# fab-jul/L3C-PyTorch

Hardware: NVIDIA B200
Metric: Mpixels/s encode+decode (lossless round-trip) (higher is better)
Workload: dtype f16

## Files before the change

### include/l3c_b200.h

```cpp
#ifndef L3C_B200_H_
#define L3C_B200_H_

#include <stddef.h>
#include <stdint.h>

#ifdef __cplusplus
extern "C" {
#endif

#define L3C_OK 0
#define L3C_EINVAL (-1)
#define L3C_ECUDA (-2)
#define L3C_EOVERFLOW (-3)
#define L3C_ENODEV (-4)
#define L3C_EUNSUPPORTED (-5)

const char *l3c_last_error(void);
int l3c_version(void);

long long l3c_launch_log(char *buf, size_t cap, int reset);


int l3c_cuda_supported(void);

int l3c_encode_cdf(const uint16_t *cdf_host, int64_t n_sym, int Lp, const int16_t *sym_host,
                   uint8_t *out_host, size_t out_cap, size_t *out_len);

int l3c_decode_cdf(const uint16_t *cdf_host, int64_t n_sym, int Lp, const uint8_t *in_host,
                   size_t in_len, int16_t *sym_out_host);

int l3c_encode_logistic_mixture(const float *targets_dev, const float *means_dev,
                                const float *log_scales_dev, const float *probs_dev, int K,
                                int64_t n_sym, int Lp, const int16_t *sym_host,
                                uint8_t *out_host, size_t out_cap, size_t *out_len);

int l3c_decode_logistic_mixture(const float *targets_dev, const float *means_dev,
                                const float *log_scales_dev, const float *probs_dev, int K,
                                int64_t n_sym, int Lp, const uint8_t *in_host, size_t in_len,
                                int16_t *sym_out_host);


typedef struct {
    const uint32_t *intervals;
    uint8_t *out;
    uint32_t n_sym;
    uint32_t out_cap;
} l3c_enc_stream_t;

int l3c_ac_encode_streams(const l3c_enc_stream_t *streams_dev, int n_streams,
                          uint32_t *out_len_dev, void *stream);

typedef struct {
    const uint16_t *table;
    const uint8_t *in;
    uint8_t *sym_out;
    uint32_t *state;
    int64_t row_pitch;
    uint32_t n_sym;
    uint32_t in_len;
} l3c_dec_stream_t;

int l3c_ac_decode_streams(const l3c_dec_stream_t *streams_dev, int n_streams, int L,
                          uint32_t first, uint32_t count, void *stream);

int l3c_pack_streams(const l3c_enc_stream_t *streams_dev, const uint32_t *len_dev,
                     const uint64_t *dst_off_dev, int n_streams, uint8_t *blob_dev, void *stream);

int l3c_lut_intervals(const uint8_t *sym_dev, const uint32_t *lut_dev, int64_t n,
                      uint32_t *intervals_dev, void *stream);


int l3c_uniform_cdf_row(int L, uint16_t *row_host);

int l3c_dmll_intervals(const float *l_dev, const uint8_t *sym_dev, const float *targets_dev,
                       int N, int HW, int C, int K, int L, int rgb, uint32_t *intervals_dev,
                       void *stream);

int l3c_dmll_build_table(const float *l_dev, const uint8_t *sym_dev, const float *targets_dev,
                         int N, int HW, int C, int K, int L, int rgb, int c, int pix0, int npix,
                         uint16_t *table_dev, int pitch, void *stream);

int l3c_dmll_build_table_tiled(const float *l_dev, const uint8_t *sym_dev, const float *targets_dev,
                               int N, int H, int W, int C, int K, int L, int rgb, int c, int th, int tw,
                               uint16_t *table_dev, int pitch, void *stream);
int l3c_reorder_tiles(const void *src_dev, void *dst_dev, int elem_bytes, int planes, int H, int W, int th,
                      int tw, int to_tiles, void *stream);

int l3c_dmll_nll(const float *l_dev, const uint8_t *sym_dev, const float *values_dev,
                 int N, int HW, int C, int K, int L, int rgb, float x_min, float x_max,
                 double *nll_dev, float *nll_map_dev ,
                 void *stream);

int l3c_dmll_channel_params(const float *l_dev, const float *x_dec_dev, int N, int HW, int C, int K,
                            int rgb, int c, float *pi_dev, float *mu_dev, float *log_scales_dev,
                            void *stream);

int l3c_dmll_sample(const float *l_dev, const float *u_sel_dev, const float *u_x_dev, int N, int HW, int C, int K,
                    int rgb, float *x_dev, void *stream);


#define L3C_CONV_RELU 1u
#define L3C_CONV_PIXEL_SHUFFLE2 2u
#define L3C_CONV_ROUND_TF32 4u

#define L3C_PREC_FP32 0
#define L3C_PREC_TF32 1
#define L3C_PREC_F16 2
#define L3C_PREC_F16X2 3

typedef struct {
    const float *x;
    const float *w;
    const float *bias;
    const float *residual;
    float *y;
    float *y_tf32;
    void *y_h;
    const void *x_h;
    const void *w_h;
    int N, H, W, Cin, x_pitch;
    int Cout, cout_pad, y_pitch, y_coff;
    int ksize, stride, dilation;
    unsigned flags;
    int precision;
    int yh_pitch;
    int yh_lo_off;
} l3c_conv_t;

int l3c_conv2d(const l3c_conv_t *p, void *stream);

int l3c_lin_dmll_intervals(const void *x_h, const void *w_h, const float *bias, const uint8_t *sym_dev,
                           const float *targets_dev, int N, int HW, int Cin, int C, int K, int L, int rgb,
                           uint32_t *intervals_dev, void *stream);

int l3c_rgb_prep(const uint8_t *img_dev, const float *A1, const float *b1, const float *A2,
                 const float *b2, int N, int HW, float *xsub_dev, float *t_dev, void *stream);

int l3c_rgb_im2col_f16(const uint8_t *img_dev, const float *A1, const float *b1, const float *A2, const float *b2,
                       int N, int H, int W, void *out_h_dev, void *stream);

int l3c_split_f16x2(const float *x_dev, long long n_px, int C, void *out_h_dev, void *stream);

int l3c_quantize_head(const float *f_dev, const float *w_dev, const float *bias_dev,
                      const float *levels_dev, int N, int HW, int Cf, int C, int L,
                      uint8_t *sym_dev, float *bnq_dev, void *stream);

int l3c_symbols_to_values(const uint8_t *sym_dev, const float *values_dev, const float *shift_dev,
                          int N, int HW, int C, int L, float *out_dev, void *stream);

int l3c_bicubic_half_u8(const uint8_t *in_dev, int N, int H, int W, uint8_t *out_dev, void *stream);

int l3c_decode_rgb_pipelined(const float *l_dev, uint8_t *sym_dev, const float *targets_dev, int N, int HW, int K,
                             int L, uint16_t *table_dev, int pitch,
                             const l3c_dec_stream_t *const *desc_dev_per_channel, int chunk_px, void *cur_stream,
                             void *const *bld_streams, void *const *dec_streams);


int l3c_partition_streams(int sm_a, int n_a, void **streams_a, int n_b, void **streams_b,
                          int *sm_a_out, int *sm_b_out);
int l3c_partition_streams2(int sm_a, int n_a, void **streams_a, int n_b_high, void **streams_b_high,
                           int n_b_low, void **streams_b_low, int *sm_a_out, int *sm_b_out);

#ifdef __cplusplus
// ... 4 lines not shown
```

### l3c_pytorch_b200/_lib.py

```python
import ctypes
import os

_HERE = os.path.dirname(os.path.abspath(__file__))
SO_PATH = os.path.join(_HERE, 'libl3c_b200.so')

c_void_p, c_int, c_int64, c_size_t, c_uint32, c_float = (
    ctypes.c_void_p, ctypes.c_int, ctypes.c_int64, ctypes.c_size_t, ctypes.c_uint32, ctypes.c_float)


class ConvDesc(ctypes.Structure):
    _fields_ = [('x', c_void_p), ('w', c_void_p), ('bias', c_void_p), ('residual', c_void_p),
                ('y', c_void_p), ('y_tf32', c_void_p), ('y_h', c_void_p), ('x_h', c_void_p), ('w_h', c_void_p),
                ('N', c_int), ('H', c_int), ('W', c_int), ('Cin', c_int), ('x_pitch', c_int),
                ('Cout', c_int), ('cout_pad', c_int), ('y_pitch', c_int), ('y_coff', c_int),
                ('ksize', c_int), ('stride', c_int), ('dilation', c_int),
                ('flags', ctypes.c_uint), ('precision', c_int), ('yh_pitch', c_int), ('yh_lo_off', c_int)]


CONV_RELU = 1
CONV_PIXEL_SHUFFLE2 = 2
CONV_ROUND_TF32 = 4
PREC_FP32, PREC_TF32, PREC_F16, PREC_F16X2 = 0, 1, 2, 3
E_UNSUPPORTED = -5
PRECISIONS = {'fp32': PREC_FP32, 'tf32': PREC_TF32, 'f16': PREC_F16, 'f16x2': PREC_F16X2}

ENC_STREAM_DTYPE = [('intervals', '<u8'), ('out', '<u8'), ('n_sym', '<u4'), ('out_cap', '<u4')]
DEC_STREAM_DTYPE = [('table', '<u8'), ('in', '<u8'), ('sym_out', '<u8'), ('state', '<u8'),
                    ('row_pitch', '<i8'), ('n_sym', '<u4'), ('in_len', '<u4')]

_SIGNATURES = {
    'l3c_last_error': (ctypes.c_char_p, []),
    'l3c_version': (c_int, []),
    'l3c_launch_log': (ctypes.c_longlong, [ctypes.c_char_p, c_size_t, c_int]),
    'l3c_cuda_supported': (c_int, []),
    'l3c_encode_cdf': (c_int, [c_void_p, c_int64, c_int, c_void_p, c_void_p, c_size_t, c_void_p]),
    'l3c_decode_cdf': (c_int, [c_void_p, c_int64, c_int, c_void_p, c_size_t, c_void_p]),
    'l3c_encode_logistic_mixture': (c_int, [c_void_p] * 4 + [c_int, c_int64, c_int, c_void_p, c_void_p,
                                                             c_size_t, c_void_p]),
    'l3c_decode_logistic_mixture': (c_int, [c_void_p] * 4 + [c_int, c_int64, c_int, c_void_p, c_size_t,
                                                             c_void_p]),
    'l3c_ac_encode_streams': (c_int, [c_void_p, c_int, c_void_p, c_void_p]),
    'l3c_ac_decode_streams': (c_int, [c_void_p, c_int, c_int, c_uint32, c_uint32, c_void_p]),
    'l3c_uniform_cdf_row': (c_int, [c_int, c_void_p]),
    'l3c_lut_intervals': (c_int, [c_void_p, c_void_p, c_int64, c_void_p, c_void_p]),
    'l3c_dmll_intervals': (c_int, [c_void_p] * 3 + [c_int] * 6 + [c_void_p, c_void_p]),
    'l3c_dmll_build_table': (c_int, [c_void_p] * 3 + [c_int] * 9 + [c_void_p, c_int, c_void_p]),
    'l3c_dmll_build_table_tiled': (c_int, [c_void_p] * 3 + [c_int] * 10 + [c_void_p, c_int, c_void_p]),
    'l3c_reorder_tiles': (c_int, [c_void_p, c_void_p] + [c_int] * 7 + [c_void_p]),
    'l3c_dmll_nll': (c_int, [c_void_p] * 3 + [c_int] * 6 + [c_float, c_float, c_void_p, c_void_p, c_void_p]),
    'l3c_dmll_channel_params': (c_int, [c_void_p, c_void_p] + [c_int] * 6 + [c_void_p] * 4),
    'l3c_dmll_sample': (c_int, [c_void_p] * 3 + [c_int] * 5 + [c_void_p, c_void_p]),
    'l3c_conv2d': (c_int, [ctypes.POINTER(ConvDesc), c_void_p]),
    'l3c_lin_dmll_intervals': (c_int, [c_void_p] * 5 + [c_int] * 7 + [c_void_p, c_void_p]),
    'l3c_rgb_prep': (c_int, [c_void_p] * 5 + [c_int, c_int, c_void_p, c_void_p, c_void_p]),
    'l3c_split_f16x2': (c_int, [c_void_p, ctypes.c_longlong, c_int, c_void_p, c_void_p]),
    'l3c_rgb_im2col_f16': (c_int, [c_void_p] * 5 + [c_int] * 3 + [c_void_p, c_void_p]),
    'l3c_quantize_head': (c_int, [c_void_p] * 4 + [c_int] * 5 + [c_void_p, c_void_p, c_void_p]),
    'l3c_symbols_to_values': (c_int, [c_void_p] * 3 + [c_int] * 4 + [c_void_p, c_void_p]),
    'l3c_bicubic_half_u8': (c_int, [c_void_p, c_int, c_int, c_int, c_void_p, c_void_p]),
    'l3c_decode_rgb_pipelined': (c_int, [c_void_p] * 3 + [c_int] * 4 + [c_void_p, c_int, c_void_p, c_int, c_void_p,
                                         c_void_p, c_void_p]),
    'l3c_pack_streams': (c_int, [c_void_p, c_void_p, c_void_p, c_int, c_void_p, c_void_p]),
    'l3c_partition_streams': (c_int, [c_int, c_int, c_void_p, c_int, c_void_p, c_void_p, c_void_p]),
    'l3c_partition_streams2': (c_int, [c_int, c_int, c_void_p, c_int, c_void_p, c_int, c_void_p, c_void_p, c_void_p]),
}

EXPORTS = sorted(_SIGNATURES)


def _bind(path):
    lib = ctypes.CDLL(path)
    for name, (restype, argtypes) in _SIGNATURES.items():
        fn = getattr(lib, name)
        fn.restype = restype
        fn.argtypes = argtypes
    return lib


def _load():
    from . import build as _build
    if not os.path.isfile(SO_PATH):
        _build.build()
    try:
        return _bind(SO_PATH)
    except AttributeError:
        _build.build(force=True)
        return _bind(SO_PATH)


lib = _load()


def check(rc):
    if rc != 0:
        msg = lib.l3c_last_error().decode('utf-8', 'replace')
        raise RuntimeError('libl3c_b200: %s (code %d)' % (msg, rc))


def cuda_supported():
    return bool(lib.l3c_cuda_supported())
```

### l3c_pytorch_b200/csrc/dmll.cu

```cuda
#include "common.cuh"
#include "dmll_math.cuh"

namespace l3c {


constexpr int IV_PIX = 64;

template <int K>
__global__ void __launch_bounds__(IV_PIX)
dmll_intervals_kernel(const float *__restrict__ l, const uint8_t *__restrict__ sym,
                      const float *__restrict__ targets, int HW, int C, int L, int rgb,
                      uint32_t *__restrict__ intervals) {
    extern __shared__ float sm[];
    const int Kp = (rgb ? 4 : 3) * C * K;
    const int pitch = Kp + 1;
    const int n = blockIdx.y;
    const int p0 = blockIdx.x * IV_PIX;
    const int np = min(IV_PIX, HW - p0);
    const float *src = l + ((size_t)n * HW + p0) * Kp;
    for (int i = threadIdx.x; i < np * Kp; i += IV_PIX) sm[(i / Kp) * pitch + (i % Kp)] = src[i];
    __syncthreads();
    if ((int)threadIdx.x >= np) return;
    const int p = p0 + threadIdx.x;
    const float *lp = sm + threadIdx.x * pitch;
    const float scale = (float)(65536 - L);
    float xr = 0.f, xg = 0.f;
    for (int c = 0; c < C; ++c) {
        ChanParams<K> cp;
        channel_params<K>(lp, 1, C, c, rgb != 0, xr, xg, cp);
        const int s = sym[((size_t)n * C + c) * HW + p];
        const uint32_t lo = mixture_cdf_u16<K>(cp.pi, cp.mu, cp.inv_s, __ldg(targets + s), scale, s);
        const uint32_t hi = (s == L - 1)
                                ? 0x10000u
                                : mixture_cdf_u16<K>(cp.pi, cp.mu, cp.inv_s, __ldg(targets + s + 1),
                                                     scale, s + 1);
        intervals[((size_t)n * C + c) * HW + p] = lo | ((hi - 1u) << 16);
        if (c == 0) xr = (float)s;
        if (c == 1) xg = (float)s;
    }
}

constexpr int TB_PIX = 256;
constexpr int TB_THREADS = 256;

__host__ __device__ __forceinline__ int tile_order_to_raster(int r, int H, int W, int th, int tw) {
    const int ty = r / (th * W);
    const int h = min(th, H - ty * th);
    const int rem = r - ty * th * W;
    const int tx = rem / (tw * h);
    const int w = min(tw, W - tx * tw);
    const int rem2 = rem - tx * tw * h;
    return (ty * th + rem2 / w) * W + tx * tw + rem2 % w;
}

template <int K>
__global__ void __launch_bounds__(TB_THREADS)
dmll_table_kernel(const float *__restrict__ l, const uint8_t *__restrict__ sym,
                  const float *__restrict__ targets, int HW, int C, int L, int rgb, int c_first,
                  int pix0, int npix, uint16_t *__restrict__ table, int pitch, int H, int W, int th, int tw) {
    __shared__ float s_pi[TB_PIX][K];
    __shared__ float s_mu[TB_PIX][K];
    __shared__ float s_is[TB_PIX][K];
    const int Kp = (rgb ? 4 : 3) * C * K;
    const int n = blockIdx.y;
    const int c = c_first + blockIdx.z;
    const int q0 = blockIdx.x * TB_PIX;
    const int np = min(TB_PIX, npix - q0);
    if ((int)threadIdx.x < np) {
        const int p = pix0 + q0 + threadIdx.x;
        const int pr = th > 0 ? tile_order_to_raster(p, H, W, th, tw) : p;
        const float *lp = l + ((size_t)n * HW + pr) * Kp;
        float xr = 0.f, xg = 0.f;
        if (rgb && c >= 1) xr = (float)sym[((size_t)n * C + 0) * HW + p];
        if (rgb && c >= 2) xg = (float)sym[((size_t)n * C + 1) * HW + p];
        ChanParams<K> cp;
        channel_params<K>(lp, 1, C, c, rgb != 0, xr, xg, cp);
#pragma unroll
        for (int k = 0; k < K; ++k) {
            s_pi[threadIdx.x][k] = cp.pi[k];
            s_mu[threadIdx.x][k] = cp.mu[k];
            s_is[threadIdx.x][k] = cp.inv_s[k];
        }
    }
    __syncthreads();
    const float scale = (float)(65536 - L);
    const int warp = threadIdx.x >> 5, lane = threadIdx.x & 31;
    const int groups = pitch >> 5;
    float tg[8];
#pragma unroll
    for (int j = 0; j < 8; ++j) {
        const int e = 32 * j + lane;
        tg[j] = (j < groups && e < L) ? __ldg(targets + e) : 0.f;
    }
    for (int r = warp; r < np; r += TB_THREADS / 32) {
        float pi[K], mu[K], is[K];
#pragma unroll
        for (int k = 0; k < K; ++k) {
            pi[k] = s_pi[r][k];
            mu[k] = s_mu[r][k];
            is[k] = s_is[r][k];
        }
        const float mu_l = s_mu[r][lane < K ? lane : 0], is_l = s_is[r][lane < K ? lane : 0];
        uint16_t *row = table + (((size_t)n * C + c) * HW + pix0 + q0 + r) * pitch;
#pragma unroll
        for (int j = 0; j < 8; ++j) {
            if (j >= groups) break;
            const int e = 32 * j + lane;
            uint32_t v = 0u;
            bool done = false;
            if (32 * j + 31 < L) {
                const float t_first = __shfl_sync(0xFFFFFFFFu, tg[j], 0), t_last = __shfl_sync(0xFFFFFFFFu, tg[j], 31);
                const float u_first = __fmul_rn(__fsub_rn(t_first, mu_l), is_l);
                const float u_last = __fmul_rn(__fsub_rn(t_last, mu_l), is_l);
                const uint32_t lo_mask = __ballot_sync(0xFFFFFFFFu, lane < K && u_first <= SAT_LO);
                const uint32_t hi_mask = __ballot_sync(0xFFFFFFFFu, lane < K && u_last >= SAT_HI);
                if ((lo_mask | hi_mask) == (1u << K) - 1u) {
                    float acc = 0.f;
#pragma unroll
                    for (int k = 0; k < K; ++k) acc = ((lo_mask >> k) & 1u) ? __fadd_rn(acc, pi[k]) : acc;
                    v = (uint32_t)(__float2int_rn(__fmul_rn(acc, scale)) + e) & 0xFFFFu;
                    done = true;
                }
            }
            if (!done) {
                const bool sat = mixture_saturated<K>(pi, mu, is, tg[j], scale, e, v);
                if (!__all_sync(0xFFFFFFFFu, sat || e >= L)) v = mixture_cdf_u16<K>(pi, mu, is, tg[j], scale, e);
            }
            row[e] = (e < L) ? (uint16_t)v : (uint16_t)0;
        }
    }
}

template <int K>
__global__ void dmll_channel_params_kernel(const float *__restrict__ l, const float *__restrict__ x_dec,
                                           int HW, int C, int rgb, int c, float *__restrict__ pi_out,
                                           float *__restrict__ mu_out, float *__restrict__ ls_out) {
    const int Kp = (rgb ? 4 : 3) * C * K;
    const int n = blockIdx.y;
    const int p = blockIdx.x * blockDim.x + threadIdx.x;
    if (p >= HW) return;
    const float *lp = l + ((size_t)n * HW + p) * Kp;
    float xr = 0.f, xg = 0.f;
    if (rgb && c >= 1) xr = x_dec[((size_t)n * C + 0) * HW + p];
    if (rgb && c >= 2) xg = x_dec[((size_t)n * C + 1) * HW + p];
    ChanParams<K> cp;
    channel_params<K>(lp, 1, C, c, rgb != 0, xr, xg, cp);
#pragma unroll
    for (int k = 0; k < K; ++k) {
        const size_t o = ((size_t)n * K + k) * HW + p;
        pi_out[o] = cp.pi[k];
        mu_out[o] = cp.mu[k];
        ls_out[o] = fmaxf(lp[2 * C * K + c * K + k], LOG_SCALES_MIN);
    }
}

__device__ __forceinline__ float softplus_f(float x) {
    return (x > 20.f) ? x : log1pf(expf(x));
}

constexpr int NLL_THREADS = 128;

template <int K>
__global__ void __launch_bounds__(NLL_THREADS)
dmll_nll_kernel(const float *__restrict__ l, const uint8_t *__restrict__ sym,
                const float *__restrict__ values, int HW, int C, int L, int rgb, float x_min,
                float x_max, double *__restrict__ partial ,
                float *__restrict__ nll_map ) {
    const int Kp = (rgb ? 4 : 3) * C * K;
    const int n = blockIdx.y;
    const int p = blockIdx.x * NLL_THREADS + threadIdx.x;
    const float half_bin = (float)(((double)x_max - (double)x_min) / (double)(L - 1) / 2.0);
    double mine = 0.0;
    if (p < HW) {
        const float *lp = l + ((size_t)n * HW + p) * Kp;
        float xr = 0.f, xg = 0.f;
        for (int c = 0; c < C; ++c) {
            const float x = __ldg(values + sym[((size_t)n * C + c) * HW + p]);
            const float *logit = lp + 0 * C * K + c * K;
            const float *mean = lp + 1 * C * K + c * K;
            const float *logs = lp + 2 * C * K + c * K;
            float lmax = logit[0];
#pragma unroll
            for (int k = 1; k < K; ++k) lmax = fmaxf(lmax, logit[k]);
            float lsum = 0.f;
#pragma unroll
            for (int k = 0; k < K; ++k) lsum += expf(logit[k] - lmax);
            const float lse_pi = lmax + logf(lsum);
            float w[K];
            float wmax = -INFINITY;
#pragma unroll
            for (int k = 0; k < K; ++k) {
                float mu = mean[k];
                if (rgb && c == 1) mu += sigmoid_rn(lp[3 * C * K + 0 * K + k]) * xr;
                if (rgb && c == 2)
                    mu += sigmoid_rn(lp[3 * C * K + 1 * K + k]) * xr +
                          sigmoid_rn(lp[3 * C * K + 2 * K + k]) * xg;
                const float inv = expf(-fmaxf(logs[k], LOG_SCALES_MIN));
                const float cx = x - mu;
                const float plus_in = inv * (cx + half_bin);
                const float min_in = inv * (cx - half_bin);
                const float delta = sigmoid_rn(plus_in) - sigmoid_rn(min_in);
                float lp_k = logf(fmaxf(delta, 1e-12f));
                if (x > x_max - 0.001f) lp_k = -softplus_f(min_in);
                if (x < x_min + 0.001f) lp_k = plus_in - softplus_f(plus_in);
                w[k] = lp_k + (logit[k] - lse_pi);
                wmax = fmaxf(wmax, w[k]);
            }
            float s = 0.f;
#pragma unroll
            for (int k = 0; k < K; ++k) s += expf(w[k] - wmax);
            const float nats = -(wmax + logf(s));
            if (nll_map) nll_map[((size_t)n * C + c) * HW + p] = nats;
            mine += (double)nats;
// ... 30 lines not shown
    const int Kp = (rgb ? 4 : 3) * C * K;
    const int n = blockIdx.y;
    const int p = blockIdx.x * blockDim.x + threadIdx.x;
    if (p >= HW) return;
    const float *lp = l + ((size_t)n * HW + p) * Kp;
    float x[3] = {0.f, 0.f, 0.f};
    int sel[3] = {0, 0, 0};
    for (int c = 0; c < C; ++c) {
        int best = 0;
        float best_v = -INFINITY;
#pragma unroll
        for (int k = 0; k < K; ++k) {
            const float u = u_sel[(((size_t)n * C + c) * K + k) * HW + p];
            const float v = lp[c * K + k] - logf(-logf(u));
            if (v > best_v) { best_v = v; best = k; }
        }
        const float mean = lp[C * K + c * K + best];
        const float ls = fmaxf(lp[2 * C * K + c * K + best], LOG_SCALES_MIN);
        const float u = u_x[((size_t)n * C + c) * HW + p];
        const float v = mean + expf(ls) * (logf(u) - logf(1.f - u));
        if (rgb) {
            sel[c] = best;
            x[c] = v;
        } else {
            x_out[((size_t)n * C + c) * HW + p] = v;
        }
    }
    if (rgb) {
        const float *co = lp + 3 * C * K;
        const float c_gr = sigmoid_rn(co[0 * K + sel[1]]);
        const float c_br = sigmoid_rn(co[1 * K + sel[2]]);
        const float c_bg = sigmoid_rn(co[2 * K + sel[2]]);
        const float x0 = fminf(fmaxf(x[0], 0.f), 255.f);
        const float x1 = fminf(fmaxf(x[1] + c_gr * x0, 0.f), 255.f);
        const float x2 = fminf(fmaxf(x[2] + c_br * x0 + c_bg * x1, 0.f), 255.f);
        x_out[((size_t)n * C + 0) * HW + p] = x0;
        x_out[((size_t)n * C + 1) * HW + p] = x1;
        x_out[((size_t)n * C + 2) * HW + p] = x2;
    }
}

static int check_common(const char *fn, int N, int HW, int C, int K, int L, int rgb) {
    L3C_REQUIRE(N >= 1 && HW >= 1, "%s: N=%d HW=%d", fn, N, HW);
    L3C_REQUIRE(K == 10, "%s: only K=10 mixtures are built (configs/ms/cr.cf:35), got K=%d", fn, K);
    L3C_REQUIRE(C >= 1 && C <= 16, "%s: C=%d", fn, C);
    L3C_REQUIRE(!rgb || C == 3, "%s: RGB coupling needs C==3 (logistic_mixture.py:236), got %d", fn, C);
    L3C_REQUIRE(L >= 2 && L <= 256, "%s: L=%d", fn, L);
    L3C_REQUIRE(N <= 65535, "%s: N=%d exceeds grid.y", fn, N);
    return L3C_OK;
}

}

extern "C" int l3c_uniform_cdf_row(int L, uint16_t *row_host) {
    using namespace l3c;
    L3C_REQUIRE(L >= 1 && L <= 256 && row_host, "l3c_uniform_cdf_row: L=%d", L);
    const float pr = 1.0f / (float)L;
    float c = 0.f;
    row_host[0] = 0;
    for (int i = 0; i < L; ++i) {
        c += pr;
        const long v = lrintf(c * 65536.0f);
        row_host[i + 1] = (uint16_t)(v & 0xFFFF);
    }
    return L3C_OK;
}

extern "C" int l3c_dmll_intervals(const float *l_dev, const uint8_t *sym_dev,
                                  const float *targets_dev, int N, int HW, int C, int K, int L,
                                  int rgb, uint32_t *intervals_dev, void *stream) {
    using namespace l3c;
    if (int e = check_common("l3c_dmll_intervals", N, HW, C, K, L, rgb)) return e;
    L3C_REQUIRE(l_dev && sym_dev && targets_dev && intervals_dev, "l3c_dmll_intervals: null pointer");
    const int Kp = (rgb ? 4 : 3) * C * K;
    const size_t smem = (size_t)IV_PIX * (Kp + 1) * sizeof(float);
    L3C_REQUIRE(smem <= 48 * 1024, "l3c_dmll_intervals: Kp=%d too large", Kp);
    dim3 grid(ceil_div(HW, IV_PIX), N);
    dmll_intervals_kernel<10><<<grid, IV_PIX, smem, (cudaStream_t)stream>>>(
        l_dev, sym_dev, targets_dev, HW, C, L, rgb, intervals_dev);
    L3C_LAUNCH_CHECK("dmll_intervals_kernel");
    return L3C_OK;
}

extern "C" int l3c_dmll_build_table(const float *l_dev, const uint8_t *sym_dev,
                                    const float *targets_dev, int N, int HW, int C, int K, int L,
                                    int rgb, int c, int pix0, int npix, uint16_t *table_dev,
                                    int pitch, void *stream) {
    using namespace l3c;
    if (int e = check_common("l3c_dmll_build_table", N, HW, C, K, L, rgb)) return e;
    L3C_REQUIRE(l_dev && targets_dev && table_dev, "l3c_dmll_build_table: null pointer");
    L3C_REQUIRE(!(rgb && c > 0) || sym_dev, "l3c_dmll_build_table: decoded symbols needed for c>0");
    L3C_REQUIRE(c < C && (c >= 0 || !rgb), "l3c_dmll_build_table: c=%d C=%d rgb=%d", c, C, rgb);
    L3C_REQUIRE((pitch == 32 && L <= 32) || (pitch == 256 && L <= 256 && L > 32),
                "l3c_dmll_build_table: pitch=%d must be 32 (L<=32) or 256, L=%d", pitch, L);
    L3C_REQUIRE(pix0 >= 0 && npix >= 0 && pix0 + npix <= HW, "l3c_dmll_build_table: pixel range");
    if (npix == 0) return L3C_OK;
    dim3 grid(ceil_div(npix, TB_PIX), N, c < 0 ? C : 1);
    dmll_table_kernel<10><<<grid, TB_THREADS, 0, (cudaStream_t)stream>>>(
        l_dev, sym_dev, targets_dev, HW, C, L, rgb, c < 0 ? 0 : c, pix0, npix, table_dev, pitch, 0, 0, 0, 0);
    L3C_LAUNCH_CHECK("dmll_table_kernel");
    return L3C_OK;
}

extern "C" int l3c_dmll_build_table_tiled(const float *l_dev, const uint8_t *sym_dev, const float *targets_dev,
                                          int N, int H, int W, int C, int K, int L, int rgb, int c, int th, int tw,
                                          uint16_t *table_dev, int pitch, void *stream) {
    using namespace l3c;
    const int HW = H * W;
    if (int e = check_common("l3c_dmll_build_table_tiled", N, HW, C, K, L, rgb)) return e;
    L3C_REQUIRE(l_dev && targets_dev && table_dev, "l3c_dmll_build_table_tiled: null pointer");
    L3C_REQUIRE(!(rgb && c > 0) || sym_dev, "l3c_dmll_build_table_tiled: decoded symbols needed for c>0");
    L3C_REQUIRE(c < C && (c >= 0 || !rgb), "l3c_dmll_build_table_tiled: c=%d C=%d rgb=%d", c, C, rgb);
    L3C_REQUIRE((pitch == 32 && L <= 32) || (pitch == 256 && L <= 256 && L > 32),
                "l3c_dmll_build_table_tiled: pitch=%d must be 32 (L<=32) or 256, L=%d", pitch, L);
    L3C_REQUIRE(th >= 1 && tw >= 1 && H >= 1 && W >= 1, "l3c_dmll_build_table_tiled: tile %dx%d", th, tw);
    dim3 grid(ceil_div(HW, TB_PIX), N, c < 0 ? C : 1);
    dmll_table_kernel<10><<<grid, TB_THREADS, 0, (cudaStream_t)stream>>>(
        l_dev, sym_dev, targets_dev, HW, C, L, rgb, c < 0 ? 0 : c, 0, HW, table_dev, pitch, H, W, th, tw);
    L3C_LAUNCH_CHECK("dmll_table_kernel");
    return L3C_OK;
}

namespace l3c {
template <typename T>
__global__ void reorder_tiles_kernel(const T *__restrict__ src, T *__restrict__ dst, int HW, int H, int W, int th,
                                     int tw, int to_tiles) {
    const int r = blockIdx.x * blockDim.x + threadIdx.x;
    if (r >= HW) return;
    const size_t base = (size_t)blockIdx.y * HW;
    const int p = tile_order_to_raster(r, H, W, th, tw);
    if (to_tiles) dst[base + r] = src[base + p];
    else dst[base + p] = src[base + r];
}
}

extern "C" int l3c_reorder_tiles(const void *src_dev, void *dst_dev, int elem_bytes, int planes, int H, int W, int th,
                                 int tw, int to_tiles, void *stream) {
    using namespace l3c;
    L3C_REQUIRE(src_dev && dst_dev && src_dev != dst_dev, "l3c_reorder_tiles: bad pointers");
    L3C_REQUIRE((elem_bytes == 1 || elem_bytes == 4) && planes >= 1 && planes <= 65535 && H >= 1 && W >= 1 && th >= 1 &&
                    tw >= 1, "l3c_reorder_tiles: bad arguments");
    const int HW = H * W;
    dim3 grid(ceil_div(HW, 256), planes);
    if (elem_bytes == 1)
        reorder_tiles_kernel<uint8_t><<<grid, 256, 0, (cudaStream_t)stream>>>((const uint8_t *)src_dev, (uint8_t *)dst_dev,
                                                                              HW, H, W, th, tw, to_tiles);
    else
        reorder_tiles_kernel<uint32_t><<<grid, 256, 0, (cudaStream_t)stream>>>((const uint32_t *)src_dev,
                                                                               (uint32_t *)dst_dev, HW, H, W, th, tw, to_tiles);
    L3C_LAUNCH_CHECK("reorder_tiles_kernel");
    return L3C_OK;
}

extern "C" int l3c_dmll_nll(const float *l_dev, const uint8_t *sym_dev, const float *values_dev,
                            int N, int HW, int C, int K, int L, int rgb, float x_min, float x_max,
                            double *nll_dev, float *nll_map_dev, void *stream) {
    using namespace l3c;
    if (int e = check_common("l3c_dmll_nll", N, HW, C, K, L, rgb)) return e;
    L3C_REQUIRE(l_dev && sym_dev && values_dev && nll_dev, "l3c_dmll_nll: null pointer");
    const int per_image = ceil_div(HW, NLL_THREADS);
    double *partial = nullptr;
    L3C_CUDA(cudaMallocAsync(&partial, sizeof(double) * (size_t)N * per_image, (cudaStream_t)stream));
    dim3 grid(per_image, N);
    dmll_nll_kernel<10><<<grid, NLL_THREADS, 0, (cudaStream_t)stream>>>(
        l_dev, sym_dev, values_dev, HW, C, L, rgb, x_min, x_max, partial, nll_map_dev);
    L3C_LAUNCH_CHECK("dmll_nll_kernel");
    nll_finish_kernel<<<N, 32, 0, (cudaStream_t)stream>>>(partial, per_image, nll_dev);
    L3C_LAUNCH_CHECK("nll_finish_kernel");
    L3C_CUDA(cudaFreeAsync(partial, (cudaStream_t)stream));
    return L3C_OK;
}

extern "C" int l3c_dmll_channel_params(const float *l_dev, const float *x_dec_dev, int N, int HW,
                                       int C, int K, int rgb, int c, float *pi_dev, float *mu_dev,
                                       float *log_scales_dev, void *stream) {
    using namespace l3c;
    if (int e = check_common("l3c_dmll_channel_params", N, HW, C, K, 256, rgb)) return e;
    L3C_REQUIRE(l_dev && pi_dev && mu_dev && log_scales_dev && c >= 0 && c < C,
                "l3c_dmll_channel_params: bad arguments");
    L3C_REQUIRE(!(rgb && c > 0) || x_dec_dev, "l3c_dmll_channel_params: decoded values needed for c>0");
    dim3 grid(ceil_div(HW, 128), N);
    dmll_channel_params_kernel<10><<<grid, 128, 0, (cudaStream_t)stream>>>(
        l_dev, x_dec_dev, HW, C, rgb, c, pi_dev, mu_dev, log_scales_dev);
    L3C_LAUNCH_CHECK("dmll_channel_params_kernel");
    return L3C_OK;
}

extern "C" int l3c_dmll_sample(const float *l_dev, const float *u_sel_dev, const float *u_x_dev, int N, int HW,
                               int C, int K, int rgb, float *x_dev, void *stream) {
    using namespace l3c;
    if (int e = check_common("l3c_dmll_sample", N, HW, C, K, 256, rgb)) return e;
    L3C_REQUIRE(l_dev && u_sel_dev && u_x_dev && x_dev, "l3c_dmll_sample: null pointer");
    dim3 grid(ceil_div(HW, 128), N);
    dmll_sample_kernel<10><<<grid, 128, 0, (cudaStream_t)stream>>>(l_dev, u_sel_dev, u_x_dev, HW, C, rgb, x_dev);
    L3C_LAUNCH_CHECK("dmll_sample_kernel");
    return L3C_OK;
}
```

### l3c_pytorch_b200/engine.py

```python
import ctypes
import os

import numpy as np
import torch

from . import _lib
from ._lib import lib, check, ConvDesc

LAUNCHES = {'n': 0}
_PRECISION = {'mode': _lib.PRECISIONS[os.environ.get('L3C_CONV_PRECISION', 'fp32')]}


def set_conv_precision(name):
    _PRECISION['mode'] = _lib.PRECISIONS[name]


def get_conv_precision():
    return {v: k for k, v in _lib.PRECISIONS.items()}[_PRECISION['mode']]


def launch_log(reset=False):
    buf = ctypes.create_string_buffer(8192)
    total = lib.l3c_launch_log(buf, len(buf), 1 if reset else 0)
    out = {}
# ... 468 lines not shown
        w = head_conv.weight.detach().float().clamp(-65504.0, 65504.0)
        cout = w.shape[0]
        assert tuple(w.shape[1:]) == (3, 3, 3) and cout % 2 == 0 and b.shape[0] <= 256
        img = torch.zeros(1, b.shape[0], 64, dtype=torch.float16, device=w.device)
        img[0, :cout, :27] = w.permute(0, 2, 3, 1).reshape(cout, 27).half()
        pc.w_im2col = img.contiguous()
    cout = head_conv.out_channels
    y_h = torch.empty(N, H, W, cout, dtype=torch.float16, device=img_u8.device)
    d = ConvDesc(x_h=cols.data_ptr(), w_h=pc.w_im2col.data_ptr(), bias=b.data_ptr(), y_h=y_h.data_ptr(),
                 N=N, H=H, W=W, Cin=64, x_pitch=64, Cout=cout, cout_pad=b.shape[0], y_pitch=cout, y_coff=0,
                 ksize=1, stride=1, dilation=1, flags=0, precision=_lib.PREC_F16)
    check(lib.l3c_conv2d(ctypes.byref(d), _stream_ptr()))
    LAUNCHES['n'] += 1
    return Act(None, y_h)


def quantize_head(f, to_q_conv, levels):
    N, H, W, Cf = f.shape
    C = to_q_conv.out_channels
    w = to_q_conv.weight.detach().float().reshape(C, Cf).t().contiguous()
    b = to_q_conv.bias.detach().float().contiguous()
    lev = levels.detach().float().contiguous()
    sym = torch.empty(N, C, H, W, dtype=torch.uint8, device=f.device)
    bnq = torch.empty(N, H, W, 8, dtype=torch.float32, device=f.device)
    check(lib.l3c_quantize_head(_ptr(f), _ptr(w), _ptr(b), _ptr(lev), N, H * W, Cf, C, lev.numel(),
                                _ptr(sym), _ptr(bnq), _stream_ptr()))
    LAUNCHES['n'] += 1
    return sym, bnq


def symbols_to_values(sym, values, shift=None):
    N, C, H, W = sym.shape
    out = torch.empty(N, H, W, 8, dtype=torch.float32, device=sym.device)
    check(lib.l3c_symbols_to_values(_ptr(sym), _ptr(values), _ptr(shift), N, H * W, C, values.numel(),
                                    _ptr(out), _stream_ptr()))
    LAUNCHES['n'] += 1
    return out


def bicubic_half(img_u8):
    N, C, H, W = img_u8.shape
    assert C == 3 and img_u8.dtype == torch.uint8 and img_u8.is_contiguous()
    out = torch.empty(N, 3, int(H * 0.5), int(W * 0.5), dtype=torch.uint8, device=img_u8.device)
    check(lib.l3c_bicubic_half_u8(_ptr(img_u8), N, H, W, _ptr(out), _stream_ptr()))
    LAUNCHES['n'] += 2
    return out


def uniform_cdf_row(L):
    row = np.zeros(L + 1, np.uint16)
    check(lib.l3c_uniform_cdf_row(L, row.ctypes.data_as(ctypes.c_void_p)))
    return row


def dmll_intervals(l, sym, targets, C, K, L, rgb):
    N, H, W, _ = l.shape
    iv = torch.empty(N, C, H * W, dtype=torch.int32, device=l.device)
    check(lib.l3c_dmll_intervals(_ptr(l), _ptr(sym), _ptr(targets), N, H * W, C, K, L, int(rgb),
                                 _ptr(iv), _stream_ptr()))
    LAUNCHES['n'] += 1
    return iv


def lut_intervals(sym, lut):
    iv = torch.empty(sym.shape[0], sym.shape[1], sym.shape[2] * sym.shape[3], dtype=torch.int32,
                     device=sym.device)
    check(lib.l3c_lut_intervals(_ptr(sym), _ptr(lut), sym.numel(), _ptr(iv), _stream_ptr()))
    LAUNCHES['n'] += 1
    return iv


def table_pitch(L):
    return 32 if L <= 32 else 256


def dmll_build_table(l, sym, targets, C, K, L, rgb, c, table, pix0=0, npix=None):
    N, H, W, _ = l.shape
    npix = H * W - pix0 if npix is None else npix
    check(lib.l3c_dmll_build_table(_ptr(l), _ptr(sym), _ptr(targets), N, H * W, C, K, L, int(rgb), c,
                                   pix0, npix, _ptr(table), table_pitch(L), _stream_ptr()))
    LAUNCHES['n'] += 1


def dmll_build_table_tiled(l, sym, targets, C, K, L, rgb, c, table, tile):
    N, H, W, _ = l.shape
    check(lib.l3c_dmll_build_table_tiled(_ptr(l), _ptr(sym), _ptr(targets), N, H, W, C, K, L, int(rgb), c,
                                         tile[0], tile[1], _ptr(table), table_pitch(L), _stream_ptr()))
    LAUNCHES['n'] += 1


def reorder_tiles(src, H, W, tile, to_tiles):
    assert src.is_contiguous() and src.dtype in (torch.uint8, torch.int32)
    planes = src.numel() // (H * W)
    dst = torch.empty_like(src)
    check(lib.l3c_reorder_tiles(_ptr(src), _ptr(dst), src.element_size(), planes, H, W, tile[0], tile[1],
                                1 if to_tiles else 0, _stream_ptr()))
    LAUNCHES['n'] += 1
    return dst


def dmll_nll(l, sym, values, C, K, L, rgb, x_min, x_max, want_map=False):
    N, H, W, _ = l.shape
    out = torch.empty(N, dtype=torch.float64, device=l.device)
    nmap = torch.empty(N, C, H, W, dtype=torch.float32, device=l.device) if want_map else None
    check(lib.l3c_dmll_nll(_ptr(l), _ptr(sym), _ptr(values), N, H * W, C, K, L, int(rgb),
                           float(x_min), float(x_max), _ptr(out), _ptr(nmap), _stream_ptr()))
    LAUNCHES['n'] += 2
    return out, nmap


def dmll_channel_params(l, x_dec, C, K, rgb, c):
    N, H, W, _ = l.shape
    outs = [torch.empty(N, K, H, W, dtype=torch.float32, device=l.device) for _ in range(3)]
    check(lib.l3c_dmll_channel_params(_ptr(l), _ptr(x_dec), N, H * W, C, K, int(rgb), c,
                                      _ptr(outs[0]), _ptr(outs[1]), _ptr(outs[2]), _stream_ptr()))
    LAUNCHES['n'] += 1
    return outs


def lin_dmll_intervals(conv, cat_h, sym, targets, C, K, L, rgb):
    N, H, W, cin = cat_h.shape
    assert cat_h.dtype == torch.float16 and cat_h.is_contiguous() and cin == conv.in_channels
    assert conv.kernel_size[0] == 1 and conv.out_channels == (4 if rgb else 3) * C * K
    w_h, b = _packed_obj(conv).get_f16()
    iv = torch.empty(N, C, H * W, dtype=torch.int32, device=cat_h.device)
    check(lib.l3c_lin_dmll_intervals(_ptr(cat_h), _ptr(w_h), _ptr(b), _ptr(sym), _ptr(targets), N, H * W, cin, C, K,
                                     L, int(rgb), _ptr(iv), _stream_ptr()))
    LAUNCHES['n'] += 1
    return iv


def dmll_sample(l, u_sel, u_x, C, K, rgb):
    N, H, W, _ = l.shape
    assert u_sel.shape == (N, C, K, H, W) and u_x.shape == (N, C, H, W)
    out = torch.empty(N, C, H, W, dtype=torch.float32, device=l.device)
    check(lib.l3c_dmll_sample(_ptr(l), _ptr(u_sel.contiguous()), _ptr(u_x.contiguous()), N, H * W, C, K, int(rgb),
                              _ptr(out), _stream_ptr()))
    LAUNCHES['n'] += 1
    return out


def _to_device_async(arr, device):
    return torch.from_numpy(np.ascontiguousarray(arr)).pin_memory().to(device, non_blocking=True)


def _desc_to_device(arr, device):
    return _to_device_async(arr.view(np.uint8).reshape(-1), device)


def ac_encode_streams(desc_np, device):
    n = desc_np.shape[0]
    desc = _desc_to_device(desc_np, device)
    lens = torch.empty(n, dtype=torch.int32, device=device)
    check(lib.l3c_ac_encode_streams(_ptr(desc), n, _ptr(lens), _stream_ptr()))
    LAUNCHES['n'] += 1
    return desc, lens


def pack_streams(desc_dev, lens_dev, dst_off_np, n, blob):
    off = _to_device_async(dst_off_np.astype(np.int64), blob.device)
    check(lib.l3c_pack_streams(_ptr(desc_dev), _ptr(lens_dev), _ptr(off), n, _ptr(blob), _stream_ptr()))
    LAUNCHES['n'] += 1


def decode_rgb_pipelined(l, S, targets, K, L, table, descs_dev, chunk_px, cur, bld, dec):
    N, H, W, _ = l.shape
# ... 20 lines not shown
```

Baseline: 94.34.

## Restructure DMLL CDF table kernel with per-group saturation ballots and vector row writes

Rewrites the CDF table builder so that for 256-wide rows each lane classifies a subset of mixture components per 32-entry group via ballots. Fully saturated groups are then filled arithmetically and written as 16-byte vectors, while only unsaturated groups evaluate sigmoids for the live components into a shared-memory row. It also pads params to 12 for float4 shared loads, caches targets in shared memory, specialises on pitch, and adds a plain reference kernel plus a shared launch helper. The aim is to cut sigmoid work and scattered 2-byte stores during table construction, at the cost of more complex warp logic and a 16-byte alignment requirement on the table.

```diff
diff --git a/include/l3c_b200.h b/include/l3c_b200.h
--- a/include/l3c_b200.h
+++ b/include/l3c_b200.h
@@ -79,6 +79,10 @@
 int l3c_dmll_build_table(const float *l_dev, const uint8_t *sym_dev, const float *targets_dev,
                          int N, int HW, int C, int K, int L, int rgb, int c, int pix0, int npix,
                          uint16_t *table_dev, int pitch, void *stream);
+
+int l3c_dmll_build_table_plain(const float *l_dev, const uint8_t *sym_dev, const float *targets_dev,
+                               int N, int HW, int C, int K, int L, int rgb, int c, int pix0, int npix,
+                               uint16_t *table_dev, int pitch, void *stream);
 
 int l3c_dmll_build_table_tiled(const float *l_dev, const uint8_t *sym_dev, const float *targets_dev,
                                int N, int H, int W, int C, int K, int L, int rgb, int c, int th, int tw,
diff --git a/l3c_pytorch_b200/_lib.py b/l3c_pytorch_b200/_lib.py
--- a/l3c_pytorch_b200/_lib.py
+++ b/l3c_pytorch_b200/_lib.py
@@ -45,6 +45,7 @@
     'l3c_lut_intervals': (c_int, [c_void_p, c_void_p, c_int64, c_void_p, c_void_p]),
     'l3c_dmll_intervals': (c_int, [c_void_p] * 3 + [c_int] * 6 + [c_void_p, c_void_p]),
     'l3c_dmll_build_table': (c_int, [c_void_p] * 3 + [c_int] * 9 + [c_void_p, c_int, c_void_p]),
+    'l3c_dmll_build_table_plain': (c_int, [c_void_p] * 3 + [c_int] * 9 + [c_void_p, c_int, c_void_p]),
     'l3c_dmll_build_table_tiled': (c_int, [c_void_p] * 3 + [c_int] * 10 + [c_void_p, c_int, c_void_p]),
     'l3c_reorder_tiles': (c_int, [c_void_p, c_void_p] + [c_int] * 7 + [c_void_p]),
     'l3c_dmll_nll': (c_int, [c_void_p] * 3 + [c_int] * 6 + [c_float, c_float, c_void_p, c_void_p, c_void_p]),
diff --git a/l3c_pytorch_b200/csrc/dmll.cu b/l3c_pytorch_b200/csrc/dmll.cu
--- a/l3c_pytorch_b200/csrc/dmll.cu
+++ b/l3c_pytorch_b200/csrc/dmll.cu
@@ -53,19 +53,47 @@
     return (ty * th + rem2 / w) * W + tx * tw + rem2 % w;
 }
 
+constexpr int TB_KP = 12;
+
 template <int K>
-__global__ void __launch_bounds__(TB_THREADS)
+__device__ __forceinline__ uint32_t cdf_entry_live(uint32_t lo, uint32_t live, const float (&pi)[K],
+                                                   const float (&mu)[K], const float (&is)[K], float t,
+                                                   float scale, int e) {
+    float sig[K];
+    bool skip[K];
+#pragma unroll
+    for (int k = 0; k < K; ++k) {
+        sig[k] = 1.0f;
+        skip[k] = !((lo >> k) & 1u);
+        if ((live >> k) & 1u) {
+            const float u = __fmul_rn(__fsub_rn(t, mu[k]), is[k]);
+            sig[k] = (u <= SAT_LO) ? 1.0f : sigmoid_from_log2(u);
+            skip[k] = u >= SAT_HI;
+        }
+    }
+    float acc = 0.f;
+#pragma unroll
+    for (int k = 0; k < K; ++k) acc = skip[k] ? acc : __fmaf_rn(pi[k], sig[k], acc);
+    return (uint32_t)(__float2int_rn(__fmul_rn(acc, scale)) + e) & 0xFFFFu;
+}
+
+template <int K, int PITCH>
+__global__ void __launch_bounds__(TB_THREADS, 3)
 dmll_table_kernel(const float *__restrict__ l, const uint8_t *__restrict__ sym,
                   const float *__restrict__ targets, int HW, int C, int L, int rgb, int c_first,
-                  int pix0, int npix, uint16_t *__restrict__ table, int pitch, int H, int W, int th, int tw) {
-    __shared__ float s_pi[TB_PIX][K];
-    __shared__ float s_mu[TB_PIX][K];
-    __shared__ float s_is[TB_PIX][K];
+                  int pix0, int npix, uint16_t *__restrict__ table, int H, int W, int th, int tw) {
+    static_assert(K <= TB_KP && TB_KP % 4 == 0 && K > 8 && K <= 12, "lanes classify terms sub, sub+4, sub+8");
+    __shared__ __align__(16) float s_pi[TB_PIX][TB_KP];
+    __shared__ __align__(16) float s_mu[TB_PIX][TB_KP];
+    __shared__ __align__(16) float s_is[TB_PIX][TB_KP];
+    __shared__ float s_t[PITCH];
+    __shared__ __align__(16) uint16_t s_row[PITCH == 256 ? TB_THREADS / 32 : 1][PITCH];
     const int Kp = (rgb ? 4 : 3) * C * K;
     const int n = blockIdx.y;
     const int c = c_first + blockIdx.z;
     const int q0 = blockIdx.x * TB_PIX;
     const int np = min(TB_PIX, npix - q0);
+    for (int e = threadIdx.x; e < PITCH; e += TB_THREADS) s_t[e] = __ldg(targets + min(e, L - 1));
     if ((int)threadIdx.x < np) {
         const int p = pix0 + q0 + threadIdx.x;
         const int pr = th > 0 ? tile_order_to_raster(p, H, W, th, tw) : p;
@@ -75,60 +103,125 @@
         if (rgb && c >= 2) xg = (float)sym[((size_t)n * C + 1) * HW + p];
         ChanParams<K> cp;
         channel_params<K>(lp, 1, C, c, rgb != 0, xr, xg, cp);
-#pragma unroll
-        for (int k = 0; k < K; ++k) {
-            s_pi[threadIdx.x][k] = cp.pi[k];
-            s_mu[threadIdx.x][k] = cp.mu[k];
-            s_is[threadIdx.x][k] = cp.inv_s[k];
+        float pi[TB_KP], mu[TB_KP], is[TB_KP];
+#pragma unroll
+        for (int k = 0; k < TB_KP; ++k) {
+            pi[k] = k < K ? cp.pi[k] : 0.f;
+            mu[k] = k < K ? cp.mu[k] : 0.f;
+            is[k] = k < K ? cp.inv_s[k] : 0.f;
+        }
+#pragma unroll
+        for (int k = 0; k < TB_KP; k += 4) {
+            *reinterpret_cast<float4 *>(&s_pi[threadIdx.x][k]) = make_float4(pi[k], pi[k + 1], pi[k + 2], pi[k + 3]);
+            *reinterpret_cast<float4 *>(&s_mu[threadIdx.x][k]) = make_float4(mu[k], mu[k + 1], mu[k + 2], mu[k + 3]);
+            *reinterpret_cast<float4 *>(&s_is[threadIdx.x][k]) = make_float4(is[k], is[k + 1], is[k + 2], is[k + 3]);
         }
     }
     __syncthreads();
     const float scale = (float)(65536 - L);
     const int warp = threadIdx.x >> 5, lane = threadIdx.x & 31;
-    const int groups = pitch >> 5;
-    float tg[8];
-#pragma unroll
-    for (int j = 0; j < 8; ++j) {
-        const int e = 32 * j + lane;
-        tg[j] = (j < groups && e < L) ? __ldg(targets + e) : 0.f;
-    }
+    const uint32_t FULL = 0xFFFFFFFFu, ALL_K = (1u << K) - 1u;
+    uint16_t *const rows = table + (((size_t)n * C + c) * HW + pix0 + q0) * PITCH;
+    const float t_lane = s_t[lane];
+    const int g = PITCH == 256 ? lane >> 2 : 0, sub = lane & 3;
+    const bool g_valid = 32 * g < L;
+    const float t_first = s_t[min(32 * g, L - 1)], t_last = s_t[min(32 * g + 31, L - 1)];
     for (int r = warp; r < np; r += TB_THREADS / 32) {
         float pi[K], mu[K], is[K];
 #pragma unroll
-        for (int k = 0; k < K; ++k) {
-            pi[k] = s_pi[r][k];
-            mu[k] = s_mu[r][k];
-            is[k] = s_is[r][k];
-        }
-        const float mu_l = s_mu[r][lane < K ? lane : 0], is_l = s_is[r][lane < K ? lane : 0];
-        uint16_t *row = table + (((size_t)n * C + c) * HW + pix0 + q0 + r) * pitch;
-#pragma unroll
-        for (int j = 0; j < 8; ++j) {
-            if (j >= groups) break;
-            const int e = 32 * j + lane;
-            uint32_t v = 0u;
-            bool done = false;
-            if (32 * j + 31 < L) {
-                const float t_first = __shfl_sync(0xFFFFFFFFu, tg[j], 0), t_last = __shfl_sync(0xFFFFFFFFu, tg[j], 31);
-                const float u_first = __fmul_rn(__fsub_rn(t_first, mu_l), is_l);
-                const float u_last = __fmul_rn(__fsub_rn(t_last, mu_l), is_l);
-                const uint32_t lo_mask = __ballot_sync(0xFFFFFFFFu, lane < K && u_first <= SAT_LO);
-                const uint32_t hi_mask = __ballot_sync(0xFFFFFFFFu, lane < K && u_last >= SAT_HI);
-                if ((lo_mask | hi_mask) == (1u << K) - 1u) {
-                    float acc = 0.f;
-#pragma unroll
-                    for (int k = 0; k < K; ++k) acc = ((lo_mask >> k) & 1u) ? __fadd_rn(acc, pi[k]) : acc;
-                    v = (uint32_t)(__float2int_rn(__fmul_rn(acc, scale)) + e) & 0xFFFFu;
-                    done = true;
+        for (int k = 0; k < TB_KP; k += 4) {
+            const float4 a = *reinterpret_cast<const float4 *>(&s_pi[r][k]);
+            const float4 b = *reinterpret_cast<const float4 *>(&s_mu[r][k]);
+            const float4 d = *reinterpret_cast<const float4 *>(&s_is[r][k]);
+            const float av[4] = {a.x, a.y, a.z, a.w}, bv[4] = {b.x, b.y, b.z, b.w}, dv[4] = {d.x, d.y, d.z, d.w};
+#pragma unroll
+            for (int i = 0; i < 4; ++i)
+                if (k + i < K) { pi[k + i] = av[i]; mu[k + i] = bv[i]; is[k + i] = dv[i]; }
+        }
+        if constexpr (PITCH == 32) {
+            const int kl = lane < K ? lane : 0;
+            const float mu_l = s_mu[r][kl], is_l = s_is[r][kl];
+            const uint32_t lo = __ballot_sync(FULL, lane < K && __fmul_rn(__fsub_rn(t_first, mu_l), is_l) <= SAT_LO);
+            const uint32_t hi = __ballot_sync(FULL, lane < K && __fmul_rn(__fsub_rn(t_last, mu_l), is_l) >= SAT_HI);
+            const uint32_t v = ((lo | hi) == ALL_K) ? cdf_entry_live<K>(lo, 0u, pi, mu, is, t_lane, scale, lane)
+                                                    : mixture_cdf_u16<K>(pi, mu, is, t_lane, scale, lane);
+            rows[(size_t)r * PITCH + lane] = lane < L ? (uint16_t)v : (uint16_t)0;
+        } else {
+            uint32_t bl[3], bh[3];
+#pragma unroll
+            for (int i = 0; i < 3; ++i) {
+                const int k = sub + 4 * i;
+                const bool ok = k < K && g_valid;
+                const float mk = s_mu[r][k], ik = s_is[r][k];
+                bl[i] = __ballot_sync(FULL, ok && __fmul_rn(__fsub_rn(t_first, mk), ik) <= SAT_LO);
+                bh[i] = __ballot_sync(FULL, ok && __fmul_rn(__fsub_rn(t_last, mk), ik) >= SAT_HI);
+            }
+            const int sh = lane & 28;
+            const uint32_t lo = ((bl[0] >> sh) & 15u) | (((bl[1] >> sh) & 15u) << 4) | (((bl[2] >> sh) & 15u) << 8);
+            const uint32_t hi = ((bh[0] >> sh) & 15u) | (((bh[1] >> sh) & 15u) << 4) | (((bh[2] >> sh) & 15u) << 8);
+            const bool sat = !g_valid || (lo | hi) == ALL_K;
+            float acc = 0.f;
+#pragma unroll
+            for (int k = 0; k < K; ++k) acc = ((lo >> k) & 1u) ? __fadd_rn(acc, pi[k]) : acc;
+            const int base = __float2int_rn(__fmul_rn(acc, scale));
+            uint32_t todo = __ballot_sync(FULL, !sat) & 0x11111111u;
+            if (todo) {
+                __syncwarp();
+                do {
+                    const int j = (__ffs(todo) - 1) >> 2;
+                    todo &= todo - 1u;
+                    const uint32_t lo_j = __shfl_sync(FULL, lo, 4 * j), hi_j = __shfl_sync(FULL, hi, 4 * j);
+                    const int e = 32 * j + lane;
+                    const uint32_t v = cdf_entry_live<K>(lo_j, ~(lo_j | hi_j) & ALL_K, pi, mu, is, s_t[e], scale, e);
+                    s_row[warp][e] = e < L ? (uint16_t)v : (uint16_t)0;
+                } while (todo);
+                __syncwarp();
+            }
+            uint4 out;
+            if (sat) {
+                const int e0 = 8 * lane, x = base + e0;
+                uint32_t w[4];
+#pragma unroll
+                for (int m = 0; m < 4; ++m) w[m] = __byte_perm(x + 2 * m, x + 2 * m + 1, 0x5410);
+                if (e0 + 8 > L) {
+#pragma unroll
+                    for (int m = 0; m < 4; ++m) {
+                        if (e0 + 2 * m >= L) w[m] = 0u;
+                        else if (e0 + 2 * m + 1 >= L) w[m] &= 0xFFFFu;
+                    }
                 }
+                out = make_uint4(w[0], w[1], w[2], w[3]);
+            } else {
+                out = *reinterpret_cast<const uint4 *>(&s_row[warp][8 * lane]);
             }
-            if (!done) {
-                const bool sat = mixture_saturated<K>(pi, mu, is, tg[j], scale, e, v);
-                if (!__all_sync(0xFFFFFFFFu, sat || e >= L)) v = mixture_cdf_u16<K>(pi, mu, is, tg[j], scale, e);
-            }
-            row[e] = (e < L) ? (uint16_t)v : (uint16_t)0;
-        }
-    }
+            *reinterpret_cast<uint4 *>(rows + (size_t)r * PITCH + 8 * lane) = out;
+        }
+    }
+}
+
+template <int K>
+__global__ void __launch_bounds__(256)
+dmll_table_plain_kernel(const float *__restrict__ l, const uint8_t *__restrict__ sym,
+                        const float *__restrict__ targets, int HW, int C, int L, int rgb, int c_first,
+                        int pix0, int npix, uint16_t *__restrict__ table, int pitch, int H, int W, int th, int tw) {
+    const long long i = (long long)blockIdx.x * blockDim.x + threadIdx.x;
+    if (i >= (long long)npix * pitch) return;
+    const int q = (int)(i / pitch), e = (int)(i % pitch);
+    const int n = blockIdx.y;
+    const int c = c_first + blockIdx.z;
+    const int p = pix0 + q;
+    const int pr = th > 0 ? tile_order_to_raster(p, H, W, th, tw) : p;
+    uint16_t v = 0;
+    if (e < L) {
+        const float *lp = l + ((size_t)n * HW + pr) * ((rgb ? 4 : 3) * C * K);
+        float xr = 0.f, xg = 0.f;
+        if (rgb && c >= 1) xr = (float)sym[((size_t)n * C + 0) * HW + p];
+        if (rgb && c >= 2) xg = (float)sym[((size_t)n * C + 1) * HW + p];
+        ChanParams<K> cp;
+        channel_params<K>(lp, 1, C, c, rgb != 0, xr, xg, cp);
+        v = (uint16_t)mixture_cdf_u16<K>(cp.pi, cp.mu, cp.inv_s, targets[e], (float)(65536 - L), e);
+    }
+    table[(((size_t)n * C + c) * HW + p) * pitch + e] = v;
 }
 
 template <int K>
@@ -325,43 +418,63 @@
     return L3C_OK;
 }
 
+namespace l3c {
+static int launch_table(const char *fn, bool plain, const float *l_dev, const uint8_t *sym_dev,
+                        const float *targets_dev, int N, int HW, int C, int K, int L, int rgb, int c, int pix0,
+                        int npix, uint16_t *table_dev, int pitch, int H, int W, int th, int tw, void *stream) {
+    if (int e = check_common(fn, N, HW, C, K, L, rgb)) return e;
+    L3C_REQUIRE(l_dev && targets_dev && table_dev, "%s: null pointer", fn);
+    L3C_REQUIRE(!(rgb && c > 0) || sym_dev, "%s: decoded symbols needed for c>0", fn);
+    L3C_REQUIRE(c < C && (c >= 0 || !rgb), "%s: c=%d C=%d rgb=%d", fn, c, C, rgb);
+    L3C_REQUIRE((pitch == 32 && L <= 32) || (pitch == 256 && L <= 256 && L > 32),
+                "%s: pitch=%d must be 32 (L<=32) or 256, L=%d", fn, pitch, L);
+    L3C_REQUIRE(pix0 >= 0 && npix >= 0 && pix0 + npix <= HW, "%s: pixel range", fn);
+    L3C_REQUIRE(plain || pitch == 32 || ((uintptr_t)table_dev & 15u) == 0,
+                "%s: table must be 16-byte aligned (rows are written as 16-byte vectors)", fn);
+    if (npix == 0) return L3C_OK;
+    cudaStream_t s = (cudaStream_t)stream;
+    const int cz = c < 0 ? C : 1, c0 = c < 0 ? 0 : c;
+    if (plain) {
+        dim3 grid((unsigned)ceil_div64((int64_t)npix * pitch, 256), N, cz);
+        dmll_table_plain_kernel<10><<<grid, 256, 0, s>>>(l_dev, sym_dev, targets_dev, HW, C, L, rgb, c0, pix0, npix,
+                                                         table_dev, pitch, H, W, th, tw);
+        L3C_LAUNCH_CHECK("dmll_table_plain_kernel");
+        return L3C_OK;
+    }
+    dim3 grid(ceil_div(npix, TB_PIX), N, cz);
+    if (pitch == 32)
+        dmll_table_kernel<10, 32><<<grid, TB_THREADS, 0, s>>>(l_dev, sym_dev, targets_dev, HW, C, L, rgb, c0, pix0,
+                                                              npix, table_dev, H, W, th, tw);
+    else
+        dmll_table_kernel<10, 256><<<grid, TB_THREADS, 0, s>>>(l_dev, sym_dev, targets_dev, HW, C, L, rgb, c0, pix0,
+                                                               npix, table_dev, H, W, th, tw);
+    L3C_LAUNCH_CHECK("dmll_table_kernel");
+    return L3C_OK;
+}
+}
+
 extern "C" int l3c_dmll_build_table(const float *l_dev, const uint8_t *sym_dev,
                                     const float *targets_dev, int N, int HW, int C, int K, int L,
                                     int rgb, int c, int pix0, int npix, uint16_t *table_dev,
                                     int pitch, void *stream) {
-    using namespace l3c;
-    if (int e = check_common("l3c_dmll_build_table", N, HW, C, K, L, rgb)) return e;
-    L3C_REQUIRE(l_dev && targets_dev && table_dev, "l3c_dmll_build_table: null pointer");
-    L3C_REQUIRE(!(rgb && c > 0) || sym_dev, "l3c_dmll_build_table: decoded symbols needed for c>0");
-    L3C_REQUIRE(c < C && (c >= 0 || !rgb), "l3c_dmll_build_table: c=%d C=%d rgb=%d", c, C, rgb);
-    L3C_REQUIRE((pitch == 32 && L <= 32) || (pitch == 256 && L <= 256 && L > 32),
-                "l3c_dmll_build_table: pitch=%d must be 32 (L<=32) or 256, L=%d", pitch, L);
-    L3C_REQUIRE(pix0 >= 0 && npix >= 0 && pix0 + npix <= HW, "l3c_dmll_build_table: pixel range");
-    if (npix == 0) return L3C_OK;
-    dim3 grid(ceil_div(npix, TB_PIX), N, c < 0 ? C : 1);
-    dmll_table_kernel<10><<<grid, TB_THREADS, 0, (cudaStream_t)stream>>>(
-        l_dev, sym_dev, targets_dev, HW, C, L, rgb, c < 0 ? 0 : c, pix0, npix, table_dev, pitch, 0, 0, 0, 0);
-    L3C_LAUNCH_CHECK("dmll_table_kernel");
-    return L3C_OK;
+    return l3c::launch_table("l3c_dmll_build_table", false, l_dev, sym_dev, targets_dev, N, HW, C, K, L, rgb, c,
+                             pix0, npix, table_dev, pitch, 0, 0, 0, 0, stream);
+}
+
+extern "C" int l3c_dmll_build_table_plain(const float *l_dev, const uint8_t *sym_dev,
+                                          const float *targets_dev, int N, int HW, int C, int K, int L,
+                                          int rgb, int c, int pix0, int npix, uint16_t *table_dev,
+                                          int pitch, void *stream) {
+    return l3c::launch_table("l3c_dmll_build_table_plain", true, l_dev, sym_dev, targets_dev, N, HW, C, K, L, rgb,
+                             c, pix0, npix, table_dev, pitch, 0, 0, 0, 0, stream);
 }
 
 extern "C" int l3c_dmll_build_table_tiled(const float *l_dev, const uint8_t *sym_dev, const float *targets_dev,
                                           int N, int H, int W, int C, int K, int L, int rgb, int c, int th, int tw,
                                           uint16_t *table_dev, int pitch, void *stream) {
-    using namespace l3c;
-    const int HW = H * W;
-    if (int e = check_common("l3c_dmll_build_table_tiled", N, HW, C, K, L, rgb)) return e;
-    L3C_REQUIRE(l_dev && targets_dev && table_dev, "l3c_dmll_build_table_tiled: null pointer");
-    L3C_REQUIRE(!(rgb && c > 0) || sym_dev, "l3c_dmll_build_table_tiled: decoded symbols needed for c>0");
-    L3C_REQUIRE(c < C && (c >= 0 || !rgb), "l3c_dmll_build_table_tiled: c=%d C=%d rgb=%d", c, C, rgb);
-    L3C_REQUIRE((pitch == 32 && L <= 32) || (pitch == 256 && L <= 256 && L > 32),
-                "l3c_dmll_build_table_tiled: pitch=%d must be 32 (L<=32) or 256, L=%d", pitch, L);
     L3C_REQUIRE(th >= 1 && tw >= 1 && H >= 1 && W >= 1, "l3c_dmll_build_table_tiled: tile %dx%d", th, tw);
-    dim3 grid(ceil_div(HW, TB_PIX), N, c < 0 ? C : 1);
-    dmll_table_kernel<10><<<grid, TB_THREADS, 0, (cudaStream_t)stream>>>(
-        l_dev, sym_dev, targets_dev, HW, C, L, rgb, c < 0 ? 0 : c, 0, HW, table_dev, pitch, H, W, th, tw);
-    L3C_LAUNCH_CHECK("dmll_table_kernel");
-    return L3C_OK;
+    return l3c::launch_table("l3c_dmll_build_table_tiled", false, l_dev, sym_dev, targets_dev, N, H * W, C, K, L,
+                             rgb, c, 0, H * W, table_dev, pitch, H, W, th, tw, stream);
 }
 
 namespace l3c {
diff --git a/l3c_pytorch_b200/engine.py b/l3c_pytorch_b200/engine.py
--- a/l3c_pytorch_b200/engine.py
+++ b/l3c_pytorch_b200/engine.py
@@ -574,6 +574,14 @@
     LAUNCHES['n'] += 1
 
 
+def dmll_build_table_plain(l, sym, targets, C, K, L, rgb, c, table, pix0=0, npix=None):
+    N, H, W, _ = l.shape
+    npix = H * W - pix0 if npix is None else npix
+    check(lib.l3c_dmll_build_table_plain(_ptr(l), _ptr(sym), _ptr(targets), N, H * W, C, K, L, int(rgb), c,
+                                         pix0, npix, _ptr(table), table_pitch(L), _stream_ptr()))
+    LAUNCHES['n'] += 1
+
+
 def dmll_build_table_tiled(l, sym, targets, C, K, L, rgb, c, table, tile):
     N, H, W, _ = l.shape
     check(lib.l3c_dmll_build_table_tiled(_ptr(l), _ptr(sym), _ptr(targets), N, H, W, C, K, L, int(rgb), c,
```

New measurement: 97.86, median of 6. +3.7%, better.
